# trzy/FasterRCNN

Hardware: AMD Instinct MI355X
Metric: images/sec (600x1000) Faster-RCNN VGG-16 inference (higher is better)
Workload: dtype f32 (float32 tensors and accumulation; 15 GEMM layers in the f32x3 split-operand emulation = two fp16 terms per block-scaled operand, three fp16 MFMAs per product; 0 in f32x6 = three bf16 terms, six bf16 MFMAs; the other 2 on exact-f32 MFMA; strict exact-f32 everywhere: config.strict_f32_images_per_

## Files before the change

### fasterrcnn_amd/_native.py

```python
import ctypes as C
import os

_HERE = os.path.dirname(os.path.abspath(__file__))
LIB_PATH = os.environ.get("FRCNN_LIB_PATH") or os.path.join(_HERE, "csrc", "libfrcnn_hip.so")

OK = 0
ABI_VERSION = 21
ERRORS = {0: "FRCNN_OK", -1: "FRCNN_EINVAL", -2: "FRCNN_EHIP", -3: "FRCNN_ENOMEM",
          -4: "FRCNN_EUNSUPPORTED", -5: "FRCNN_ENODEVICE"}
RELU = 1
POOL2 = 2
NUM_KCLASS = 11
KCLASS_NAMES = ("conv3x3_mfma", "conv3x3_c3", "linear_mfma", "proposals", "roi_pool", "other", "winograd_transforms",
                "winograd_gemm", "winograd_x6_transforms", "winograd_x6_gemm", "winograd_x3f")

SYMBOLS = (
    "frcnn_abi_version", "frcnn_error_string", "frcnn_last_hip_error", "frcnn_device_count",
    "frcnn_anchors", "frcnn_pack_conv3x3", "frcnn_pack_conv3x3_c3", "frcnn_pack_fc_chw_to_hwc",
    "frcnn_pack_stack_rows", "frcnn_conv3x3_c3", "frcnn_conv3x3_c3_cmax", "frcnn_conv3x3_workspace_bytes", "frcnn_conv3x3_nhwc",
    "frcnn_maxpool2x2_nhwc",
    "frcnn_linear_workspace_bytes", "frcnn_linear", "frcnn_softmax_rows", "frcnn_rpn_proposals",
    "frcnn_nms", "frcnn_roi_pool", "frcnn_roi_pool_x3t", "frcnn_detections", "frcnn_ctx_create", "frcnn_ctx_create_proposals", "frcnn_ctx_destroy",
    "frcnn_ctx_bytes", "frcnn_vgg16_forward", "frcnn_ctx_tensor", "frcnn_ctx_timing_enable",
    "frcnn_ctx_timing_read",
    "frcnn_output_block_layout", "frcnn_stream_depend", "frcnn_ctx_submit_stats", "frcnn_predict_submit", "frcnn_streams_share_queue",
    "frcnn_fold_bn_pack", "frcnn_conv_workspace_bytes", "frcnn_conv_nhwc", "frcnn_conv_nhwc_math", "frcnn_conv_nhwc_x3g", "frcnn_conv_nhwc_x3g_tickets", "frcnn_pack_conv_x3g_weights", "frcnn_x3_saturation_events", "frcnn_tensor_absmax", "frcnn_conv7x7_s2_c3",
    "frcnn_maxpool3x3_s2_nhwc", "frcnn_spatial_mean_nhwc", "frcnn_resnet_forward", "frcnn_rpn_targets",
    "frcnn_preprocess_workspace_bytes", "frcnn_preprocess",
    "frcnn_conv3x3_uses_winograd", "frcnn_resnet_block_uses_winograd", "frcnn_pack_conv3x3_winograd",
    "frcnn_pack_conv3x3_winograd_taps", "frcnn_conv3x3_winograd_workspace_bytes",
    "frcnn_conv3x3_nhwc_winograd",
    "frcnn_conv3x3_uses_winograd_fused", "frcnn_resnet_block_uses_winograd_fused", "frcnn_pack_conv3x3_winograd_fused", "frcnn_pack_conv3x3_winograd_fused_taps",
    "frcnn_conv3x3_nhwc_winograd_fused",
    "frcnn_roi_align", "frcnn_roi_align_backward",
    "frcnn_x6t_record_bytes", "frcnn_split_rows_x6t", "frcnn_gemm_x6t_workspace_bytes", "frcnn_gemm_x6t", "frcnn_split_pixels_x6t", "frcnn_split_patches3x3_x6t",
    "frcnn_conv3x3_uses_winograd_x6", "frcnn_conv3x3_winograd_x6_pack_bytes", "frcnn_pack_conv3x3_winograd_x6",
    "frcnn_conv3x3_winograd_x6_workspace_bytes", "frcnn_conv3x3_nhwc_winograd_x6",
    "frcnn_pixel_absmax", "frcnn_split_pixels_x3t", "frcnn_split_patches3x3_x3t",
    "frcnn_x3t_blob_bytes", "frcnn_pack_rows_x3t", "frcnn_conv3x3_winograd_x3_pack_bytes", "frcnn_pack_conv3x3_winograd_x3",
    "frcnn_conv3x3_winograd_x3_workspace_bytes", "frcnn_conv3x3_nhwc_winograd_x3",
    "frcnn_conv3x3_winograd_x3_fused_workspace_bytes", "frcnn_conv3x3_nhwc_winograd_x3_fused", "frcnn_conv3x3_nhwc_winograd_x3_chain",
    "frcnn_x3t_record_bytes", "frcnn_rows_scale_x3t", "frcnn_split_rows_x3t", "frcnn_gemm_x3t_workspace_bytes", "frcnn_gemm_x3t",
    "frcnn_conv3x3_nhwc_winograd_fused_maps", "frcnn_ctx_create_backbone", "frcnn_resnet_backbone", "frcnn_resnet_forward_features", "frcnn_resnet_rpn_roipool", "frcnn_ctx_create_head", "frcnn_resnet_head",
    "frcnn_label_proposals", "frcnn_gather_rows", "frcnn_rpn_loss", "frcnn_detector_loss",
    "frcnn_gemm_tn_math", "frcnn_conv3x3_wgrad_math", "frcnn_conv_wgrad_math", "frcnn_bottleneck_backward_workspace_bytes", "frcnn_bottleneck_backward",
    "frcnn_gemm_tn_workspace_bytes", "frcnn_gemm_tn", "frcnn_conv3x3_wgrad_workspace_bytes", "frcnn_conv3x3_wgrad",
    "frcnn_pack_conv3x3_dgrad", "frcnn_relu_backward", "frcnn_dropout", "frcnn_dropout_relu_backward", "frcnn_add_inplace", "frcnn_maxpool2x2_backward",
    "frcnn_roi_pool_backward_workspace_bytes", "frcnn_roi_pool_backward", "frcnn_transpose", "frcnn_sgd_step", "frcnn_sgd_step_fold",
    "frcnn_conv_wgrad_workspace_bytes", "frcnn_conv_wgrad", "frcnn_conv_dgrad_workspace_bytes", "frcnn_conv_dgrad", "frcnn_conv_dgrad_math",
    "frcnn_pack_conv_dgrad", "frcnn_scale_rows", "frcnn_bn_scale_shift", "frcnn_spatial_mean_backward",
    "frcnn_ops_roi_align", "frcnn_ops_roi_align_backward", "frcnn_ops_roi_pool", "frcnn_ops_roi_pool_backward",
    "frcnn_ops_nms_workspace_bytes", "frcnn_ops_nms",
    "frcnn_ops_ms_roi_align", "frcnn_ops_ms_roi_align_workspace_bytes", "frcnn_ops_ms_roi_align_backward",
    "frcnn_ops_half_run", "frcnn_ops_roi_align_16", "frcnn_ops_roi_align_backward_16", "frcnn_ops_roi_pool_16",
    "frcnn_ops_roi_pool_backward_16", "frcnn_ops_ms_roi_align_16", "frcnn_ops_ms_roi_align_backward_16",
    "frcnn_ops_ps_roi_pool", "frcnn_ops_ps_roi_pool_backward", "frcnn_ops_ps_roi_align", "frcnn_ops_ps_roi_align_backward",
    "frcnn_ops_ps_roi_pool_16", "frcnn_ops_ps_roi_pool_backward_16", "frcnn_ops_ps_roi_align_16", "frcnn_ops_ps_roi_align_backward_16",
    "frcnn_ops_deform_workspace_bytes", "frcnn_ops_deform_forward", "frcnn_ops_deform_backward_columns", "frcnn_ops_deform_backward_offset",
    "frcnn_ops_deform_input_plan", "frcnn_ops_deform_backward_input", "frcnn_ops_deform_backward_weight",
    "frcnn_ops_deform_roi_pool_cull_list", "frcnn_ops_deform_roi_pool_workspace_bytes", "frcnn_ops_deform_roi_pool",
    "frcnn_ops_deform_roi_pool_backward", "frcnn_ops_deform_roi_pool_16", "frcnn_ops_deform_roi_pool_backward_16",
    "frcnn_ops_box_iou_rotated", "frcnn_ops_nms_rotated", "frcnn_ops_roi_align_rotated_cull_list", "frcnn_ops_roi_align_rotated",
    "frcnn_ops_roi_align_rotated_backward", "frcnn_ops_roi_align_rotated_16", "frcnn_ops_roi_align_rotated_backward_16",
    "frcnn_ops_carafe_max_kernel", "frcnn_ops_carafe_channel_chunk", "frcnn_ops_carafe_tile_width", "frcnn_ops_carafe_tile_height",
    "frcnn_ops_carafe", "frcnn_ops_carafe_backward", "frcnn_ops_carafe_16", "frcnn_ops_carafe_backward_16",
# ... 282 lines not shown
    "frcnn_spatial_mean_nhwc": (C.c_int, [_vp, _vp, _i, _i, _i, _i, _vp]),
    "frcnn_resnet_forward": (C.c_int, [_vp, C.POINTER(ResNetWeights), C.POINTER(ForwardParams), _vp, _i, _i,
                                       _vp, _vp, _vp, _vp, _vp, _vp, _vp]),
    "frcnn_resnet_forward_features": (C.c_int, [_vp, C.POINTER(ResNetWeights), C.POINTER(ForwardParams), _vp, _i, _i,
                                                _vp, _vp, _vp, _vp, _vp, _vp, _vp]),
    "frcnn_resnet_backbone": (C.c_int, [_vp, C.POINTER(ResNetWeights), C.POINTER(ForwardParams), _vp, _i, _i, _i, _vp, _vp]),
    "frcnn_pixel_absmax": (C.c_int, [_vp, _vp, C.c_longlong, _i, _vp]),
    "frcnn_split_pixels_x3t": (C.c_int, [_vp, _vp, _vp, _vp, _i, _i, _i, _i, _i, _i, _vp]),
    "frcnn_split_patches3x3_x3t": (C.c_int, [_vp, _vp, _vp, _vp, _i, _i, _i, _i, _i, _i, _vp]),
    "frcnn_x3t_blob_bytes": (C.c_size_t, [_i, _i, _i]),
    "frcnn_pack_rows_x3t": (C.c_int, [_vp, _i, _sz, _vp, _i, _i, _i, _i, _vp]),
    "frcnn_conv3x3_winograd_x3_pack_bytes": (C.c_size_t, [_i, _i]),
    "frcnn_pack_conv3x3_winograd_x3": (C.c_int, [_vp, _vp, _i, _i, _vp]),
    "frcnn_conv3x3_winograd_x3_workspace_bytes": (C.c_size_t, [_i, _i, _i, _i, _i]),
    "frcnn_conv3x3_nhwc_winograd_x3": (C.c_int, [_vp, _vp, _vp, _vp, _i, _i, _i, _i, _i, _u, _vp, _sz, _vp]),
    "frcnn_conv3x3_winograd_x3_fused_workspace_bytes": (C.c_size_t, [_i, _i, _i]),
    "frcnn_conv3x3_nhwc_winograd_x3_fused": (C.c_int, [_vp, _vp, _vp, _vp, _i, _i, _i, _i, _i, _u, _vp, _sz, _vp]),
    "frcnn_conv3x3_nhwc_winograd_x3_chain": (C.c_int, [_vp, _vp, _vp, _vp, _i, _i, _i, _i, _i, _u, _i, _vp, _sz, _vp, _vp, _vp]),
    "frcnn_x3t_record_bytes": (C.c_size_t, [_i, _i]),
    "frcnn_rows_scale_x3t": (C.c_int, [_vp, _i, _sz, _vp, _i, _i, _i, _i, _vp]),
    "frcnn_split_rows_x3t": (C.c_int, [_vp, _i, _sz, _vp, _vp, _i, _i, _i, _i, _vp]),
    "frcnn_gemm_x3t_workspace_bytes": (C.c_size_t, [_i, _i, _i, _i]),
    "frcnn_gemm_x3t": (C.c_int, [_vp, _vp, _i, _sz, _sz, _vp, _vp, _i, _sz, _sz, _vp, _vp, _vp, _i, _sz, _i, _i, _i, _i, _u, _vp, _sz, _vp]),
    "frcnn_ctx_create_backbone": (C.c_int, [C.POINTER(C.c_void_p), _i, _i, _i]),
    "frcnn_ctx_create_head": (C.c_int, [C.POINTER(C.c_void_p), _i]),
    "frcnn_resnet_rpn_roipool": (C.c_int, [_vp, C.POINTER(ResNetWeights), C.POINTER(ForwardParams), _vp, _i, _i, _vp, _vp, _vp, _vp, _vp, _vp]),
    "frcnn_resnet_head": (C.c_int, [_vp, C.POINTER(ResNetWeights), C.POINTER(ForwardParams), _vp, _i, _vp, _vp, _vp]),
    "frcnn_conv3x3_nhwc_winograd_fused_maps": (C.c_int, [_vp, _vp, _vp, _vp, _i, _i, _i, _i, _i, _u, _vp]),
    "frcnn_label_proposals": (C.c_int, [_vp, _vp, _i, _vp, _vp, _i, _i, _f, _f, C.POINTER(C.c_float), C.POINTER(C.c_float),
                                        _vp, _vp, _vp, _vp, _vp, _vp]),
    "frcnn_gather_rows": (C.c_int, [_vp, _vp, _i, _i, _vp, _vp]),
    "frcnn_rpn_loss": (C.c_int, [_vp, _i, _i, _vp, _i, _vp, _vp, _vp, _vp]),
    "frcnn_detector_loss": (C.c_int, [_vp, _vp, _vp, _vp, _i, _i, _vp, _vp, _i, _vp]),
    "frcnn_gemm_tn_workspace_bytes": (C.c_size_t, [_i, _i, _i]),
    "frcnn_gemm_tn": (C.c_int, [_vp, _i, _vp, _i, _vp, _i, _i, _i, _i, _vp, _sz, _vp]),
    "frcnn_gemm_tn_math": (C.c_int, [_vp, _i, _vp, _i, _vp, _i, _i, _i, _i, _i, _vp, _sz, _vp]),
    "frcnn_conv3x3_wgrad_math": (C.c_int, [_vp, _vp, _vp, _i, _i, _i, _i, _i, _vp, _sz, _vp]),
    "frcnn_conv_wgrad_math": (C.c_int, [_vp, _vp, _vp, _i, _i, _i, _i, _i, _i, _i, _i, _i, _vp, _sz, _vp]),
    "frcnn_bottleneck_backward_workspace_bytes": (C.c_int, [_vp, _vp, _vp, _vp, _i, _i, _i, _i, _i, C.POINTER(C.c_size_t), C.POINTER(C.c_size_t)]),
    "frcnn_bottleneck_backward": (C.c_int, [_vp, _vp, _vp, _vp, _vp, _vp, _vp, _vp, _vp, _vp, _vp, _vp, _vp, _i, _i, _i, _i, _i, _i, _vp, _sz, _vp, _sz,
                                            _vp, _vp]),
    "frcnn_conv3x3_wgrad_workspace_bytes": (C.c_size_t, [_i, _i, _i, _i]),
    "frcnn_conv3x3_wgrad": (C.c_int, [_vp, _vp, _vp, _i, _i, _i, _i, _vp, _sz, _vp]),
    "frcnn_pack_conv3x3_dgrad": (C.c_int, [_vp, _vp, _i, _i, _vp]),
    "frcnn_conv_wgrad_workspace_bytes": (C.c_size_t, [_i] * 8),
    "frcnn_conv_wgrad": (C.c_int, [_vp, _vp, _vp, _i, _i, _i, _i, _i, _i, _i, _i, _vp, _sz, _vp]),
# ... 95 lines not shown
```

### fasterrcnn_amd/csrc/api.hip

```cpp
#include "common.h"
#include <algorithm>
#include <cmath>
#include <cstring>
#include <string>
#include <vector>
#include <new>

namespace frcnn {

static thread_local std::string g_hip_error;
void set_hip_error(hipError_t e) { g_hip_error = hipGetErrorString(e); }

static size_t align_up(size_t v, size_t a) { return (v + a - 1) / a * a; }

struct EventRec { int cls; hipEvent_t start, stop; };

}

using namespace frcnn;

struct frcnn_ctx {
    int max_h = 0, max_w = 0, max_rois = 0, max_images = 0;
    int max_fh = 0, max_fw = 0, a_cap = 0, pre_cap = 0;
    void* slab = nullptr;
// ... 267 lines not shown
    if (!d_a || !d_inv_scale) return FRCNN_EINVAL;
    return launch_rows_scale_x3t(d_a, lda, a_batch_floats, d_inv_scale, rows, rows_padded, K, batches, as_stream(stream));
}

int frcnn_split_rows_x3t(const float* d_a, int lda, size_t a_batch_floats, const float* d_inv_scale, void* d_rec, int rows, int rows_padded,
                         int K, int batches, void* stream)
{
    if (!d_a || !d_rec || !d_inv_scale) return FRCNN_EINVAL;
    return launch_split_rows_x3t(d_a, lda, a_batch_floats, d_inv_scale, d_rec, rows, rows_padded, K, batches, as_stream(stream));
}

size_t frcnn_gemm_x3t_workspace_bytes(int M, int N, int K, int batches) { return gemm_x3t_workspace_bytes(M, N, K, batches); }

int frcnn_gemm_x3t(const void* d_a_rec, const float* d_a_inv, int a_rows, size_t a_batch_bytes, size_t a_inv_batch_floats,
                   const void* d_b_rec, const float* d_b_inv, int b_rows, size_t b_batch_bytes, size_t b_inv_batch_floats,
                   const float* d_bias, const float* d_residual, float* d_c, int ldc, size_t c_batch_floats, int M, int N, int K,
                   int batches, unsigned flags, void* d_ws, size_t ws_bytes, void* stream)
{
    return launch_gemm_x3t(d_a_rec, d_a_inv, a_rows, a_batch_bytes, a_inv_batch_floats, d_b_rec, d_b_inv, b_rows, b_batch_bytes,
                           b_inv_batch_floats, d_bias, d_residual, d_c, ldc, c_batch_floats, M, N, K, batches, flags, d_ws, ws_bytes,
                           as_stream(stream));
}

size_t frcnn_conv3x3_winograd_x3_fused_workspace_bytes(int n_maps, int H, int W)
{
    return n_maps > 0 && H > 0 && W > 0 ? conv3x3_winograd_x3_fused_workspace_bytes(n_maps, H, W) : 0;
}

int frcnn_conv3x3_nhwc_winograd_x3_fused(const float* d_x, const void* d_blob, const float* d_bias, float* d_y, int n_maps, int H, int W,
                                         int cin, int cout, unsigned flags, void* d_ws, size_t ws_bytes, void* stream)
{
    if (!d_x || !d_blob || !d_bias || !d_y) return FRCNN_EINVAL;
    return launch_conv3x3_winograd_x3_fused(d_x, d_blob, d_bias, d_y, n_maps, H, W, cin, cout, flags, d_ws, ws_bytes, as_stream(stream));
}

int frcnn_pixel_absmax(const float* d_x, float* d_cmax, long long pixels, int c, void* stream)
{
    if (!d_x || !d_cmax) return FRCNN_EINVAL;
    return launch_pixel_absmax(d_x, d_cmax, pixels, c, as_stream(stream));
}

int frcnn_split_pixels_x3t(const float* d_x, const float* d_cmax, void* d_rec, float* d_inv_scale, int n_maps, int H, int W, int c, int stride,
                           int rows_padded, void* stream)
{
    if (!d_x || !d_rec) return FRCNN_EINVAL;
    return launch_split_pixels_x3t(d_x, d_cmax, d_rec, d_inv_scale, n_maps, H, W, c, stride, rows_padded, as_stream(stream));
// ... 1024 lines not shown

    const int R_ = p->post_nms;
    const bool fc_x6t = p->fc_math_mode == FRCNN_FC_F32X6T;
    const bool fc_x3t = p->fc_math_mode == FRCNN_FC_F32X3T;
    if (fc_x6t || fc_x3t) { rc = ensure_fc_records(c, s); if (rc) return rc; }
    if (fc_x3t) {
        const int rr = c->rec_rows;
        const size_t w1rec = x3t_record_bytes(4096, 49 * 512), w2rec = x3t_record_bytes(4096, 4096);
        const float* w1inv = reinterpret_cast<const float*>(reinterpret_cast<const unsigned char*>(w->fc1_w) + w1rec);
        const float* w2inv = reinterpret_cast<const float*>(reinterpret_cast<const unsigned char*>(w->fc2_w) + w2rec);
        if (p->roi_op == FRCNN_ROI_ALIGN) {
            STEP(4, launch_roi_align(c->fm, fh, fw, 512, d_props, d_counts + 2, R_, 7, 1.0f / 16.0f, p->roi_sampling_ratio, 0, c->roi_out, s));
            STEP(2, launch_rows_scale_x3t(c->roi_out, 49 * 512, 0, c->roi_inv, R_, rr, 49 * 512, 1, s));
            STEP(2, launch_split_rows_x3t(c->roi_out, 49 * 512, 0, c->roi_inv, c->roi_rec, R_, rr, 49 * 512, 1, s));
        } else {
            STEP(4, launch_roi_pool_x3t(c->fm, fh, fw, 512, d_props, d_counts + 2, R_, 7, 1.0f / 16.0f,
                                        fm_cmax_ready ? const_cast<float*>(fm_cmax_ready) : c->fm_cmax, c->roi_inv, c->roi_rec, rr, s, fm_cmax_ready != nullptr));
        }
        STEP(2, launch_gemm_x3t(c->roi_rec, c->roi_inv, rr, 0, 0, w->fc1_w, w1inv, 4096, 0, 0, w->fc1_b, nullptr, c->fc1_out, 4096, 0, R_, 4096,
                                49 * 512, 1, R, c->lin_ws, c->lin_ws_bytes, s, 0));
        STEP(2, launch_rows_scale_x3t(c->fc1_out, 4096, 0, c->fc1_inv, R_, rr, 4096, 1, s));
        STEP(2, launch_split_rows_x3t(c->fc1_out, 4096, 0, c->fc1_inv, c->fc1_rec, R_, rr, 4096, 1, s));
        STEP(2, launch_gemm_x3t(c->fc1_rec, c->fc1_inv, rr, 0, 0, w->fc2_w, w2inv, 4096, 0, 0, w->fc2_b, nullptr, c->fc2_out, 4096, 0, R_, 4096,
                                4096, 1, R, c->lin_ws, c->lin_ws_bytes, s, 2));
    } else
    if (fc_x6t) {
        const int rr = c->rec_rows;
        if (p->roi_op == FRCNN_ROI_ALIGN) {
            STEP(4, launch_roi_align(c->fm, fh, fw, 512, d_props, d_counts + 2, R_, 7, 1.0f / 16.0f, p->roi_sampling_ratio, 0, c->roi_out, s));
            STEP(2, launch_split_rows_x6t(c->roi_out, 49 * 512, 0, c->roi_rec, R_, rr, 49 * 512, 1, s));
        } else {
            STEP(4, launch_roi_pool_x6t(c->fm, fh, fw, 512, d_props, d_counts + 2, R_, 7, 1.0f / 16.0f, c->roi_rec, rr, s));
        }
        static const int fc_tiles = []() { const char* e = frcnn_knob("FRCNN_FC_TILES"); return e ? atoi(e) : 0; }();
        STEP(2, launch_gemm_x6t(c->roi_rec, rr, 0, w->fc1_w, 4096, 0, w->fc1_b, nullptr, c->fc1_out, 4096, 0, R_, 4096, 49 * 512, 1, R,
                                c->lin_ws, c->lin_ws_bytes, s, fc_tiles));
        STEP(2, launch_split_rows_x6t(c->fc1_out, 4096, 0, c->fc1_rec, R_, rr, 4096, 1, s));
        STEP(2, launch_gemm_x6t(c->fc1_rec, rr, 0, w->fc2_w, 4096, 0, w->fc2_b, nullptr, c->fc2_out, 4096, 0, R_, 4096, 4096, 1, R,
                                c->lin_ws, c->lin_ws_bytes, s, fc_tiles));
    } else
    {
        if (p->roi_op == FRCNN_ROI_ALIGN) {
            STEP(4, launch_roi_align(c->fm, fh, fw, 512, d_props, d_counts + 2, R_, 7, 1.0f / 16.0f, p->roi_sampling_ratio, 0, c->roi_out, s));
        } else {
            STEP(4, launch_roi_pool(c->fm, fh, fw, 512, d_props, d_counts + 2, R_, 7, 1.0f / 16.0f, c->roi_out, s));
        }
        STEP(2, launch_linear(c->roi_out, 49 * 512, w->fc1_w, w->fc1_b, c->fc1_out, 4096, R_, 4096, 49 * 512, R,
// ... 641 lines not shown
```

### fasterrcnn_amd/csrc/gemm_x3t.hip

```cpp
#include "x3t.h"

namespace frcnn {

typedef _Float16 hx_f16x8 __attribute__((ext_vector_type(8)));

#ifndef HX_ABLATE
#define HX_ABLATE 0
#endif
__global__ __launch_bounds__(256)
void rows_scale_x3t_kernel(const float* __restrict__ a, int lda, size_t a_batch, float* __restrict__ inv_scale, int R, int rows_padded,
                           int K, int batches)
{
    const int lane = threadIdx.x & 63;
    const long long wave = (long long)blockIdx.x * 4 + (threadIdx.x >> 6);
    if (wave >= (long long)batches * rows_padded) return;
    const int row = (int)(wave % rows_padded), batch = (int)(wave / rows_padded);
    float mx = 0.f;
    if (row < R) {
        const float* src = a + (size_t)batch * a_batch + (size_t)row * lda;
        for (int k = 4 * lane; k < K; k += 256) {
            const f32x4 v = *reinterpret_cast<const f32x4*>(src + k);
            mx = fmaxf(fmaxf(mx, fmaxf(fabsf(v[0]), fabsf(v[1]))), fmaxf(fabsf(v[2]), fabsf(v[3])));
        }
    }
// ... 179 lines not shown
    int nchunks, chunks_per_split, splits, batches;
    int mtiles, ntiles;
    int relu;
    int total;
};

template <int WTM, int WTN, int WVM, int WVN, int NSUB>
struct HxCfg {
    static constexpr int NW = WVM * WVN, THREADS = 64 * NW;
    static constexpr int ARB = WVM * WTM, BRB = WVN * WTN;
    static constexpr int BM = 32 * ARB, BN = 32 * BRB;
    static constexpr int A_BYTES = ARB * HX_RB, B_BYTES = BRB * HX_RB;
    static constexpr int STAGE1 = A_BYTES + B_BYTES;
    static constexpr int STAGE = NSUB * STAGE1;
    static constexpr int NBUF = NSUB == 1 ? 3 : 2;
    static constexpr int DIST = NBUF - 1;
    static constexpr size_t LDS_BYTES = NBUF * (size_t)STAGE;
    static constexpr int NPA = ARB * 2, NPB = BRB * 2, NP = NPA + NPB;
    static constexpr int PPW = (NSUB * NP + NW - 1) / NW;
};

typedef __attribute__((address_space(3))) void* hx_lds_ptr;

template <int WTM, int WTN, int WVM, int WVN, int NSUB>
__global__ __launch_bounds__(64 * WVM * WVN, 2)
void gemm_x3t_kernel(const HxParams p)
{
    using C = HxCfg<WTM, WTN, WVM, WVN, NSUB>;
    extern __shared__ __attribute__((aligned(16))) unsigned char smem_hx[];
    const int tid = threadIdx.x, lane = tid & 63;
    const int wave = __builtin_amdgcn_readfirstlane(tid >> 6);
    const int wm = wave / WVN, wn = wave % WVN;

    int bid = blockIdx.x;
    {
        const int q = p.total >> 3, r = p.total & 7, xcd = bid & 7, idx = bid >> 3;
        bid = (xcd < r ? xcd * (q + 1) : r * (q + 1) + (xcd - r) * q) + idx;
    }
    const int nt = bid % p.ntiles;
    int t = bid / p.ntiles;
    const int mt = t % p.mtiles;
    t /= p.mtiles;
    const int split = t % p.splits;
    const int batch = t / p.splits;

    const int c_begin = split * p.chunks_per_split;
    int c_end = c_begin + p.chunks_per_split;
    if (c_end > p.nchunks) c_end = p.nchunks;
    const int nst = (c_end - c_begin) / NSUB;

    const size_t a_chunk = (size_t)p.a_rbt * HX_RB, b_chunk = (size_t)p.b_rbt * HX_RB;
    const unsigned char* ag = p.a + (size_t)batch * p.a_batch + (size_t)mt * C::A_BYTES + (size_t)c_begin * a_chunk + lane * 16;
    const unsigned char* bg = p.b + (size_t)batch * p.b_batch + (size_t)nt * C::B_BYTES + (size_t)c_begin * b_chunk + lane * 16;

    auto issue_stage = [&](int s, int buf) {
        const unsigned char* as = ag + (size_t)s * NSUB * a_chunk;
        const unsigned char* bs = bg + (size_t)s * NSUB * b_chunk;
        unsigned char* ldsb = smem_hx + buf * C::STAGE;
#pragma unroll
        for (int i = 0; i < C::PPW; ++i) {
            int q = wave + C::NW * i;
            q = q < NSUB * C::NP ? q : NSUB * C::NP - 1;
            const int sub = q / C::NP, r = q - sub * C::NP;
            const unsigned char* src = r < C::NPA ? as + sub * a_chunk + r * HX_PIECE : bs + sub * b_chunk + (r - C::NPA) * HX_PIECE;
            __builtin_amdgcn_global_load_lds(src, (hx_lds_ptr)(ldsb + sub * C::STAGE1 + r * HX_PIECE), 16, 0, 0);
        }
    };
    f32x16 acc[WTM][WTN];
#pragma unroll
    for (int i = 0; i < WTM; ++i)
#pragma unroll
        for (int j = 0; j < WTN; ++j)
#pragma unroll
            for (int r = 0; r < 16; ++r) acc[i][j][r] = 0.f;

    hx_f16x8 ah[WTM], al[WTM], bh[WTN], bl[WTN];
#pragma unroll
    for (int i = 0; i < WTM; ++i)
#pragma unroll
        for (int e = 0; e < 8; ++e) al[i][e] = (_Float16)0.f;
#pragma unroll
    for (int j = 0; j < WTN; ++j)
#pragma unroll
        for (int e = 0; e < 8; ++e) bh[j][e] = (_Float16)0.f;

#ifndef HX_NO_SCHED
#define HX_NO_SCHED 0
#endif
#define HX_SGB(mask, n) __builtin_amdgcn_sched_group_barrier(mask, n, 0)
#define HX_TERM(A, B)                                                                                  \
    _Pragma("unroll") for (int i = 0; i < WTM; ++i)                                                     \
        _Pragma("unroll") for (int j = 0; j < WTN; ++j)                                                 \
            if (!(HX_ABLATE & 2)) acc[i][j] = __builtin_amdgcn_mfma_f32_32x32x16_f16(B[j], A[i], acc[i][j], 0, 0, 0);

#ifdef HX_CLOCKS
    unsigned long long clk0 = 0, real0 = 0, clk1 = 0, real1 = 0;
    const unsigned long long real_entry = __builtin_amdgcn_s_memrealtime();
#endif
    if (nst > 0) {
        issue_stage(0, 0);
        if (C::DIST == 2) issue_stage(nst > 1 ? 1 : 0, 1);
        asm volatile("s_waitcnt vmcnt(%0)" ::"n"((C::DIST - 1) * C::PPW) : "memory");
        __builtin_amdgcn_s_barrier();
        int cur = 0;
        const int a_off = wm * WTM * HX_RB + lane * 16;
        const int b_off = C::A_BYTES + wn * WTN * HX_RB + lane * 16;
#ifdef HX_CLOCKS
        clk0 = __builtin_readcyclecounter(); real0 = __builtin_amdgcn_s_memrealtime();
#endif
        for (int s = 0; s < nst; ++s) {
            const int nxt = C::NBUF == 3 ? (cur == 0 ? 2 : cur - 1) : (cur ^ 1);
#pragma unroll
            for (int sub = 0; sub < NSUB; ++sub) {
                const unsigned char* at = smem_hx + cur * C::STAGE + sub * C::STAGE1 + a_off;
                const unsigned char* bt = smem_hx + cur * C::STAGE + sub * C::STAGE1 + b_off;
                if (!(HX_ABLATE & 16) || s == 0) {
#pragma unroll
                for (int i = 0; i < WTM; ++i) ah[i] = *reinterpret_cast<const hx_f16x8*>(at + i * HX_RB);
#pragma unroll
                for (int j = 0; j < WTN; ++j) bl[j] = *reinterpret_cast<const hx_f16x8*>(bt + j * HX_RB + HX_PIECE);
                }
                if (sub == 0 && !(HX_ABLATE & 1)) issue_stage(s + C::DIST < nst ? s + C::DIST : nst - 1, nxt);
                HX_TERM(al, bh)
                HX_TERM(ah, bl)
                if (!(HX_ABLATE & 16) || s == 0) {
#pragma unroll
                for (int j = 0; j < WTN; ++j) bh[j] = *reinterpret_cast<const hx_f16x8*>(bt + j * HX_RB);
#pragma unroll
                for (int i = 0; i < WTM; ++i) al[i] = *reinterpret_cast<const hx_f16x8*>(at + i * HX_RB + HX_PIECE);
                }
                HX_TERM(ah, bh)
#if !HX_NO_SCHED && !HX_ABLATE
// ... 2 lines not shown
                if (sub == 0) {
                    _Pragma("unroll") for (int q = 0; q < (PW < NT ? PW : NT); ++q) { HX_SGB(0x008, 1); HX_SGB(0x010, 1); }
                    if (PW > NT) HX_SGB(0x010, PW - NT);
                    if (NT > PW) HX_SGB(0x008, NT - PW);
                } else {
                    HX_SGB(0x008, NT);
                }
                _Pragma("unroll") for (int q = 0; q < (NF < NT ? NF : NT); ++q) { HX_SGB(0x008, 1); HX_SGB(0x100, 1); }
                if (NF > NT) HX_SGB(0x100, NF - NT);
                if (NT > NF) HX_SGB(0x008, NT - NF);
                HX_SGB(0x008, NT);
#endif
            }
            __builtin_amdgcn_sched_barrier(0);
            asm volatile("s_waitcnt vmcnt(%0) lgkmcnt(0)" ::"n"((C::DIST - 1) * C::PPW) : "memory");
            __builtin_amdgcn_s_barrier();
            cur = cur == C::NBUF - 1 ? 0 : cur + 1;
            __builtin_amdgcn_sched_barrier(0);
        }
#ifdef HX_CLOCKS
        clk1 = __builtin_readcyclecounter(); real1 = __builtin_amdgcn_s_memrealtime();
#endif
        HX_TERM(al, bh)
        asm volatile("s_waitcnt vmcnt(0)" ::: "memory");
    }
#undef HX_TERM
#undef HX_SGB

    const bool direct = p.splits == 1;
    float* dst;
    int ldd;
    if (direct) { dst = p.c + (size_t)batch * p.c_batch; ldd = p.ldc; }
    else        { dst = p.ws + ((size_t)split * p.batches + batch) * (size_t)p.M * p.N; ldd = p.N; }
    const int m_base = mt * C::BM + 32 * WTM * wm + (lane & 31);
    const int n_base = nt * C::BN + 32 * WTN * wn + 4 * (lane >> 5);
    const float* ainv = p.a_inv + (size_t)batch * p.a_inv_batch;
    const float* binv = p.b_inv + (size_t)batch * p.b_inv_batch;
#pragma unroll
    for (int i = 0; i < WTM; ++i) {
        const int m = m_base + 32 * i;
        if (m >= p.M) continue;
        const float sa = ainv[m];
        float* row = dst + (size_t)m * ldd;
#pragma unroll
        for (int j = 0; j < WTN; ++j) {
#pragma unroll
            for (int g = 0; g < 4; ++g) {
                const int n = n_base + 32 * j + 8 * g;
                if (n >= p.N) continue;
                const f32x4 sb = *reinterpret_cast<const f32x4*>(binv + n);
                f32x4 v;
#pragma unroll
                for (int e = 0; e < 4; ++e) v[e] = (acc[i][j][4 * g + e] * sa) * sb[e];
                if (direct && p.bias != nullptr) v = v + *reinterpret_cast<const f32x4*>(p.bias + n);
                if (direct && p.residual != nullptr)
                    v = v + *reinterpret_cast<const f32x4*>(p.residual + (size_t)batch * p.c_batch + (size_t)m * ldd + n);
                if (direct && p.relu) {
#pragma unroll
                    for (int e = 0; e < 4; ++e) v[e] = fmaxf(v[e], 0.f);
                }
                if (HX_ABLATE & 4) asm volatile("" ::"v"(v));
                else *reinterpret_cast<f32x4*>(row + n) = v;
            }
        }
    }
#ifdef HX_CLOCKS
    if (lane == 0 && p.ws != nullptr) {
        const unsigned long long real_exit = __builtin_amdgcn_s_memrealtime();
        float* o = p.ws + ((size_t)blockIdx.x * C::NW + wave) * 8;
        o[0] = (float)(clk1 - clk0); o[1] = (float)(real1 - real0); o[2] = (float)(real0 - real_entry); o[3] = (float)(real_exit - real1);
        o[4] = (float)nst; o[5] = (float)(real_entry & 0xFFFFFF); o[6] = (float)(real_exit & 0xFFFFFF); o[7] = 1.0f;
    }
#endif
}

size_t x3t_record_bytes(int rows_padded, int K) { return (size_t)(K / 16) * (rows_padded / 32) * HX_RB; }

int launch_rows_scale_x3t(const float* a, int lda, size_t a_batch_floats, float* inv_scale, int R, int rows_padded, int K, int batches,
                          hipStream_t s)
{
    if (R < 1 || rows_padded < R || rows_padded % 32 != 0 || K < 16 || K % 16 != 0 || lda < K || lda % 4 != 0 || batches < 1)
        return FRCNN_EINVAL;
    const long long waves = (long long)batches * rows_padded;
    const long long blocks = (waves + 3) / 4;
    if (blocks > 0x7fffffffLL) return FRCNN_EINVAL;
    hipLaunchKernelGGL(rows_scale_x3t_kernel, dim3((unsigned)blocks), dim3(256), 0, s, a, lda, a_batch_floats, inv_scale, R, rows_padded, K,
                       batches);
// ... 31 lines not shown
    return check_launch();
}

int launch_split_patches3x3_x3t(const float* x, const float* cmax, void* rec, float* inv, int N, int H, int W, int C, int stride,
                                int rows_padded, hipStream_t s)
{
    if (N < 1 || H < 1 || W < 1 || C < 16 || C % 16 != 0 || stride < 1 || stride > 2 || rows_padded % 32 != 0 || !cmax || !inv) return FRCNN_EINVAL;
    const int Ho = (H - 1) / stride + 1, Wo = (W - 1) / stride + 1;
    const long long R = (long long)N * Ho * Wo;
    if (R > rows_padded || R > 0x7fffffffLL) return FRCNN_EINVAL;
    const long long waves = (long long)(9 * C / 16) * (rows_padded / 32);
    hipLaunchKernelGGL(split_patches3x3_x3t_kernel, dim3((unsigned)((waves + 3) / 4)), dim3(256), 0, s, x, cmax,
                       static_cast<unsigned char*>(rec), inv, H, W, Ho, Wo, C, stride, (int)R, rows_padded / 32, 9 * C / 16);
    return check_launch();
}

struct HxPlan { int cfg, mtiles, ntiles, splits, chunks_per_split; };

static HxPlan plan_gemm_x3t(int M, int N, int K, int batches, int tiles_mode = -1)
{
    HxPlan pl;
    const int chunks = K / 16;
    static const int env_force = []() { const char* e = frcnn_knob("FRCNN_HX_CFG"); return e ? atoi(e) : -1; }();
    const int mode = tiles_mode >= 0 ? tiles_mode : gemm_x6t_get_tiles();
    const int force = (env_force >= 0 && tiles_mode < 0) ? env_force : (mode == 1 ? 0 : mode == 2 ? 1 : -1);
    const long long u0 = (long long)cdiv(M, 320) * cdiv(N, 256) * batches;
    const long long u1 = (long long)cdiv(M, 160) * cdiv(N, 128) * batches;
    int splits0 = 1;
    while (u0 * splits0 * 2 <= 256 && chunks / (splits0 * 2) >= 8) splits0 *= 2;
    const double c0 = (double)((u0 * splits0 + 255) / 256) * 1920.0 / splits0 + (splits0 > 1 ? 600.0 : 0.0);
    int splits1 = 1;
    while (u1 * splits1 * 2 <= 256 && chunks / (splits1 * 2) >= 8) splits1 *= 2;
    const double c1 = (double)((u1 * splits1 + 255) / 256) * 480.0 / 0.85 / splits1 + (splits1 > 1 ? 600.0 : 0.0);
    pl.cfg = (force == 0 || force == 1) ? force : (c1 < c0 ? 1 : 0);
    static const bool big_unsplit = frcnn_knob("FRCNN_HX_BIG_UNSPLIT") != nullptr;
    if (big_unsplit && force < 0 && pl.cfg == 1 && splits1 == 1) { pl.cfg = 0; splits0 = 1; }
    int splits = pl.cfg == 1 ? splits1 : splits0;
    if (splits > chunks) splits = chunks;
    pl.mtiles = pl.cfg == 1 ? cdiv(M, 160) : cdiv(M, 320);
    pl.ntiles = pl.cfg == 1 ? cdiv(N, 128) : cdiv(N, 256);
    pl.chunks_per_split = cdiv(chunks, splits);
    pl.splits = cdiv(chunks, pl.chunks_per_split);
    return pl;
}

size_t gemm_x3t_workspace_bytes(int M, int N, int K, int batches)
// ... 20 lines not shown
    const HxPlan pl = plan_gemm_x3t(M, N, K, batches, tiles_mode);
    if (pl.splits > 1 && (ws == nullptr || ws_bytes < (size_t)pl.splits * batches * M * N * sizeof(float))) return FRCNN_EINVAL;
    HxParams p;
    p.a = static_cast<const unsigned char*>(a_rec);
    p.b = static_cast<const unsigned char*>(b_rec);
    p.a_inv = a_inv; p.b_inv = b_inv;
    p.c = c;
    p.ws = static_cast<float*>(ws);
    p.bias = bias;
    p.residual = residual;
    p.a_batch = a_batch_bytes; p.b_batch = b_batch_bytes; p.c_batch = c_batch_floats;
    p.a_inv_batch = a_inv_batch; p.b_inv_batch = b_inv_batch;
    p.a_rbt = a_rows / 32; p.b_rbt = b_rows / 32;
    p.M = M; p.N = N; p.ldc = ldc;
    p.nchunks = K / 16; p.chunks_per_split = pl.chunks_per_split; p.splits = pl.splits; p.batches = batches;
    p.mtiles = pl.mtiles; p.ntiles = pl.ntiles;
    p.relu = (flags & FRCNN_RELU) ? 1 : 0;
    const long long total = (long long)pl.mtiles * pl.ntiles * batches * pl.splits;
    if (total > 0x7fffffffLL) return FRCNN_EINVAL;
    p.total = (int)total;
    static const int env_nsub = []() { const char* e = frcnn_knob("FRCNN_HX_NSUB"); return e ? atoi(e) : 0; }();
    const int last = p.nchunks - (pl.splits - 1) * pl.chunks_per_split;
    const bool even = pl.chunks_per_split % 2 == 0 && last % 2 == 0;
    const int nsub = !even ? 1 : (env_nsub == 1 || env_nsub == 2) ? env_nsub : (pl.chunks_per_split >= 64 ? 2 : 1);
#define HX_LAUNCH(TM, TN, VM, VN, NS)                                                                          \
    do {                                                                                                      \
        using C = HxCfg<TM, TN, VM, VN, NS>;                                                                    \
        auto kern = gemm_x3t_kernel<TM, TN, VM, VN, NS>;                                                        \
        FRCNN_MAX_LDS_ONCE(kern, C::LDS_BYTES);                                                                 \
        hipLaunchKernelGGL(kern, dim3((unsigned)total), dim3(C::THREADS), C::LDS_BYTES, s, p);                  \
    } while (0)
    if (pl.cfg == 1) { if (nsub == 2) HX_LAUNCH(5, 1, 1, 4, 2); else HX_LAUNCH(5, 1, 1, 4, 1); }
    else             { if (nsub == 2) HX_LAUNCH(5, 2, 2, 4, 2); else HX_LAUNCH(5, 2, 2, 4, 1); }
#undef HX_LAUNCH
    int rc = check_launch();
    if (rc || pl.splits == 1) return rc;
    return launch_gemm_x6t_reduce(static_cast<const float*>(ws), bias, residual, c, ldc, c_batch_floats, M, N, batches, pl.splits, p.relu, s);
}

}
```

### fasterrcnn_amd/csrc/x3t.h

```cpp
#pragma once
#include "common.h"

namespace frcnn {

static constexpr int HX_PIECE = 1024;
static constexpr int HX_RB = 2 * HX_PIECE;

__device__ __forceinline__ unsigned hx_pack2(_Float16 a, _Float16 b)
{
    return (unsigned)__builtin_bit_cast(unsigned short, a) | ((unsigned)__builtin_bit_cast(unsigned short, b) << 16);
}

__device__ __forceinline__ void hx_split8(const float (&v)[8], uint4& ph, uint4& pl)
{
    _Float16 hi[8], lo[8];
#pragma unroll
    for (int j = 0; j < 8; ++j) {
        const float vj = v[j] > 65504.f ? 65504.f : (v[j] < -65504.f ? -65504.f : v[j]);
        hi[j] = (_Float16)vj;
        lo[j] = (_Float16)(vj - (float)hi[j]);
    }
    ph = make_uint4(hx_pack2(hi[0], hi[1]), hx_pack2(hi[2], hi[3]), hx_pack2(hi[4], hi[5]), hx_pack2(hi[6], hi[7]));
    pl = make_uint4(hx_pack2(lo[0], lo[1]), hx_pack2(lo[2], lo[3]), hx_pack2(lo[4], lo[5]), hx_pack2(lo[6], lo[7]));
}

__device__ __forceinline__ void hx_row_scale(float mx, float& mult, float& inv)
{
    int e = 0;
    if (mx > 0.f) {
// ... 12 lines not shown
```

### include/frcnn_hip.h

```cpp
#ifndef FRCNN_HIP_H
#define FRCNN_HIP_H

#include <stddef.h>
#include <stdint.h>

#ifdef __cplusplus
extern "C" {
#endif

#define FRCNN_OK            0
#define FRCNN_EINVAL       -1
#define FRCNN_EHIP         -2
#define FRCNN_ENOMEM       -3
#define FRCNN_EUNSUPPORTED -4
#define FRCNN_ENODEVICE    -5

#define FRCNN_ABI_VERSION 21

#define FRCNN_RELU   1u
#define FRCNN_POOL2  2u
#define FRCNN_X3G_WSPLIT 0x800u

int         frcnn_abi_version(void);
const char* frcnn_error_string(int code);
// ... 64 lines not shown
int frcnn_pack_rows_x3t(const float* d_a, int lda, size_t a_batch_floats, void* d_blob, int rows, int rows_padded, int K, int batches,
                        void* stream);
size_t frcnn_conv3x3_winograd_x3_pack_bytes(int cout, int cin);
int frcnn_pack_conv3x3_winograd_x3(const float* d_u_f32, void* d_blob, int cout, int cin, void* stream);
size_t frcnn_conv3x3_winograd_x3_workspace_bytes(int n_maps, int H, int W, int cin, int cout);
int frcnn_conv3x3_nhwc_winograd_x3(const float* d_x, const void* d_blob, const float* d_bias, float* d_y, int n_maps, int H, int W, int cin,
                                   int cout, unsigned flags, void* d_ws, size_t ws_bytes, void* stream);
size_t frcnn_conv3x3_winograd_x3_fused_workspace_bytes(int n_maps, int H, int W);
int frcnn_conv3x3_nhwc_winograd_x3_fused(const float* d_x, const void* d_blob, const float* d_bias, float* d_y, int n_maps, int H, int W,
                                         int cin, int cout, unsigned flags, void* d_ws, size_t ws_bytes, void* stream);
int frcnn_conv3x3_nhwc_winograd_x3_chain(const float* d_x, const void* d_blob, const float* d_bias, float* d_y, int n_maps, int H, int W, int cin,
                                         int cout, unsigned flags, int one_launch, void* d_ws, size_t ws_bytes, const float* d_cmax_in,
                                         float* d_cmax_out, void* stream);
size_t frcnn_x3t_record_bytes(int rows_padded, int K);
int frcnn_rows_scale_x3t(const float* d_a, int lda, size_t a_batch_floats, float* d_inv_scale, int rows, int rows_padded, int K, int batches,
                         void* stream);
int frcnn_split_rows_x3t(const float* d_a, int lda, size_t a_batch_floats, const float* d_inv_scale, void* d_rec, int rows, int rows_padded,
                         int K, int batches, void* stream);
size_t frcnn_gemm_x3t_workspace_bytes(int M, int N, int K, int batches);
int frcnn_gemm_x3t(const void* d_a_rec, const float* d_a_inv, int a_rows, size_t a_batch_bytes, size_t a_inv_batch_floats,
                   const void* d_b_rec, const float* d_b_inv, int b_rows, size_t b_batch_bytes, size_t b_inv_batch_floats,
                   const float* d_bias, const float* d_residual, float* d_c, int ldc, size_t c_batch_floats, int M, int N, int K,
                   int batches, unsigned flags, void* d_ws, size_t ws_bytes, void* stream);

int frcnn_split_pixels_x6t(const float* d_x, void* d_rec, int N, int H, int W, int C, int stride, int rows_padded, void* stream);
int frcnn_conv3x3_uses_winograd_x6(int cin, int cout);
size_t frcnn_conv3x3_winograd_x6_pack_bytes(int cout, int cin);
int frcnn_pack_conv3x3_winograd_x6(const float* d_w_oihw, const float* d_row_scale, void* d_u_rec, int cout, int cin, void* stream);
size_t frcnn_conv3x3_winograd_x6_workspace_bytes(int n_maps, int H, int W, int cin, int cout);
int frcnn_conv3x3_nhwc_winograd_x6(const float* d_x, const void* d_u_rec, const float* d_bias, float* d_y, int n_maps, int H, int W, int cin,
                                   int cout, unsigned flags, void* d_ws, size_t ws_bytes, void* stream);
int frcnn_split_patches3x3_x6t(const float* d_x, void* d_rec, int N, int H, int W, int C, int stride, int rows_padded, void* stream);
int frcnn_maxpool2x2_nhwc(const float* d_x, float* d_y, int H, int W, int c, void* stream);

int frcnn_fold_bn_pack(const float* d_w_oihw, const float* d_gamma, const float* d_beta,
                       const float* d_mean, const float* d_var, float eps, int cout, int cin, int ksize,
                       float* d_w_packed, float* d_b_packed, void* stream);
size_t frcnn_conv_workspace_bytes(int N, int H, int W, int cin, int cout, int ksize, int stride, int pad);
int frcnn_conv_nhwc(const float* d_x, const float* d_w_packed, const float* d_bias, const float* d_residual,
                    float* d_y, int N, int H, int W, int cin, int cout, int ksize, int stride, int pad,
                    unsigned flags, void* d_ws, size_t ws_bytes, void* stream);
int frcnn_conv7x7_s2_c3(const float* d_x_chw, const float* d_w_packed, const float* d_bias, float* d_y,
                        int H, int W, int cout, unsigned flags, void* stream);
int frcnn_maxpool3x3_s2_nhwc(const float* d_x, float* d_y, int H, int W, int c, void* stream);
int frcnn_spatial_mean_nhwc(const float* d_x, float* d_y, int N, int H, int W, int c, void* stream);

// ... 459 lines not shown
```

Before: 980.3.

## Add 16x16x32 f16 MFMA path for x3t GEMM and use it for fc2

Adds a K32 variant of the x3t split-fp16 GEMM kernel that issues 16x16x32 f16 MFMAs over both 16-k chunks of a stage, using 4-wide accumulators and a new fragment-offset layout. It software-pipelines the global-to-LDS loads between MFMA groups. The fc2 layer call switches to tiles mode 4 to select this path, and a new API entry point exposes the tile mode. This gives higher MFMA throughput per instruction and better overlap, at the cost of more accumulator registers and a new epilogue mapping.

```diff
diff --git a/fasterrcnn_amd/_native.py b/fasterrcnn_amd/_native.py
--- a/fasterrcnn_amd/_native.py
+++ b/fasterrcnn_amd/_native.py
@@ -41,6 +41,7 @@
     "frcnn_conv3x3_winograd_x3_workspace_bytes", "frcnn_conv3x3_nhwc_winograd_x3",
     "frcnn_conv3x3_winograd_x3_fused_workspace_bytes", "frcnn_conv3x3_nhwc_winograd_x3_fused", "frcnn_conv3x3_nhwc_winograd_x3_chain",
     "frcnn_x3t_record_bytes", "frcnn_rows_scale_x3t", "frcnn_split_rows_x3t", "frcnn_gemm_x3t_workspace_bytes", "frcnn_gemm_x3t",
+    "frcnn_gemm_x3t_tiles", "frcnn_x3t_frag16_offset",
     "frcnn_conv3x3_nhwc_winograd_fused_maps", "frcnn_ctx_create_backbone", "frcnn_resnet_backbone", "frcnn_resnet_forward_features", "frcnn_resnet_rpn_roipool", "frcnn_ctx_create_head", "frcnn_resnet_head",
     "frcnn_label_proposals", "frcnn_gather_rows", "frcnn_rpn_loss", "frcnn_detector_loss",
     "frcnn_gemm_tn_math", "frcnn_conv3x3_wgrad_math", "frcnn_conv_wgrad_math", "frcnn_bottleneck_backward_workspace_bytes", "frcnn_bottleneck_backward",
@@ -369,6 +370,8 @@
     "frcnn_split_rows_x3t": (C.c_int, [_vp, _i, _sz, _vp, _vp, _i, _i, _i, _i, _vp]),
     "frcnn_gemm_x3t_workspace_bytes": (C.c_size_t, [_i, _i, _i, _i]),
     "frcnn_gemm_x3t": (C.c_int, [_vp, _vp, _i, _sz, _sz, _vp, _vp, _i, _sz, _sz, _vp, _vp, _vp, _i, _sz, _i, _i, _i, _i, _u, _vp, _sz, _vp]),
+    "frcnn_gemm_x3t_tiles": (C.c_int, [_vp, _vp, _i, _sz, _sz, _vp, _vp, _i, _sz, _sz, _vp, _vp, _vp, _i, _sz, _i, _i, _i, _i, _u, _vp, _sz, _vp, _i]),
+    "frcnn_x3t_frag16_offset": (C.c_int, [_i, _i, _i]),
     "frcnn_ctx_create_backbone": (C.c_int, [C.POINTER(C.c_void_p), _i, _i, _i]),
     "frcnn_ctx_create_head": (C.c_int, [C.POINTER(C.c_void_p), _i]),
     "frcnn_resnet_rpn_roipool": (C.c_int, [_vp, C.POINTER(ResNetWeights), C.POINTER(ForwardParams), _vp, _i, _i, _vp, _vp, _vp, _vp, _vp, _vp]),
diff --git a/fasterrcnn_amd/csrc/api.hip b/fasterrcnn_amd/csrc/api.hip
--- a/fasterrcnn_amd/csrc/api.hip
+++ b/fasterrcnn_amd/csrc/api.hip
@@ -1,4 +1,5 @@
 #include "common.h"
+#include "x3t.h"
 #include <algorithm>
 #include <cmath>
 #include <cstring>
@@ -313,6 +314,23 @@
                            as_stream(stream));
 }
 
+int frcnn_gemm_x3t_tiles(const void* d_a_rec, const float* d_a_inv, int a_rows, size_t a_batch_bytes, size_t a_inv_batch_floats,
+                         const void* d_b_rec, const float* d_b_inv, int b_rows, size_t b_batch_bytes, size_t b_inv_batch_floats,
+                         const float* d_bias, const float* d_residual, float* d_c, int ldc, size_t c_batch_floats, int M, int N, int K,
+                         int batches, unsigned flags, void* d_ws, size_t ws_bytes, void* stream, int tiles_mode)
+{
+    if (tiles_mode < -1 || tiles_mode > 4) return FRCNN_EINVAL;
+    return launch_gemm_x3t(d_a_rec, d_a_inv, a_rows, a_batch_bytes, a_inv_batch_floats, d_b_rec, d_b_inv, b_rows, b_batch_bytes,
+                           b_inv_batch_floats, d_bias, d_residual, d_c, ldc, c_batch_floats, M, N, K, batches, flags, d_ws, ws_bytes,
+                           as_stream(stream), tiles_mode);
+}
+
+int frcnn_x3t_frag16_offset(int lane, int half, int stage1_bytes)
+{
+    if (lane < 0 || lane > 63 || half < 0 || half > 1 || stage1_bytes < HX_RB || stage1_bytes % HX_RB != 0) return -1;
+    return hx_frag16_offset(lane, stage1_bytes) + 256 * half;
+}
+
 size_t frcnn_conv3x3_winograd_x3_fused_workspace_bytes(int n_maps, int H, int W)
 {
     return n_maps > 0 && H > 0 && W > 0 ? conv3x3_winograd_x3_fused_workspace_bytes(n_maps, H, W) : 0;
@@ -1383,7 +1401,7 @@
         STEP(2, launch_rows_scale_x3t(c->fc1_out, 4096, 0, c->fc1_inv, R_, rr, 4096, 1, s));
         STEP(2, launch_split_rows_x3t(c->fc1_out, 4096, 0, c->fc1_inv, c->fc1_rec, R_, rr, 4096, 1, s));
         STEP(2, launch_gemm_x3t(c->fc1_rec, c->fc1_inv, rr, 0, 0, w->fc2_w, w2inv, 4096, 0, 0, w->fc2_b, nullptr, c->fc2_out, 4096, 0, R_, 4096,
-                                4096, 1, R, c->lin_ws, c->lin_ws_bytes, s, 2));
+                                4096, 1, R, c->lin_ws, c->lin_ws_bytes, s, 4));
     } else
     if (fc_x6t) {
         const int rr = c->rec_rows;
diff --git a/fasterrcnn_amd/csrc/gemm_x3t.hip b/fasterrcnn_amd/csrc/gemm_x3t.hip
--- a/fasterrcnn_amd/csrc/gemm_x3t.hip
+++ b/fasterrcnn_amd/csrc/gemm_x3t.hip
@@ -225,10 +225,11 @@
 
 typedef __attribute__((address_space(3))) void* hx_lds_ptr;
 
-template <int WTM, int WTN, int WVM, int WVN, int NSUB>
+template <int WTM, int WTN, int WVM, int WVN, int NSUB, bool K32 = false>
 __global__ __launch_bounds__(64 * WVM * WVN, 2)
 void gemm_x3t_kernel(const HxParams p)
 {
+    static_assert(!K32 || NSUB == 2, "the 16x16x32 body reads both chunks of a 32-k stage");
     using C = HxCfg<WTM, WTN, WVM, WVN, NSUB>;
     extern __shared__ __attribute__((aligned(16))) unsigned char smem_hx[];
     const int tid = threadIdx.x, lane = tid & 63;
@@ -269,21 +270,31 @@
             __builtin_amdgcn_global_load_lds(src, (hx_lds_ptr)(ldsb + sub * C::STAGE1 + r * HX_PIECE), 16, 0, 0);
         }
     };
-    f32x16 acc[WTM][WTN];
+    constexpr int MT = 2 * WTM, NT = 2 * WTN;
+    f32x16 acc[K32 ? 1 : WTM][K32 ? 1 : WTN];
+    f32x4 acc4[K32 ? MT : 1][K32 ? NT : 1];
+    if constexpr (K32) {
+#pragma unroll
+        for (int i = 0; i < MT; ++i)
+#pragma unroll
+            for (int j = 0; j < NT; ++j) acc4[i][j] = f32x4{0.f, 0.f, 0.f, 0.f};
+    } else {
 #pragma unroll
     for (int i = 0; i < WTM; ++i)
 #pragma unroll
         for (int j = 0; j < WTN; ++j)
 #pragma unroll
             for (int r = 0; r < 16; ++r) acc[i][j][r] = 0.f;
-
-    hx_f16x8 ah[WTM], al[WTM], bh[WTN], bl[WTN];
-#pragma unroll
-    for (int i = 0; i < WTM; ++i)
+    }
+
+    constexpr int FM = K32 ? MT : WTM, FN = K32 ? NT : WTN;
+    hx_f16x8 ah[FM], al[FM], bh[FN], bl[FN];
+#pragma unroll
+    for (int i = 0; i < FM; ++i)
 #pragma unroll
         for (int e = 0; e < 8; ++e) al[i][e] = (_Float16)0.f;
 #pragma unroll
-    for (int j = 0; j < WTN; ++j)
+    for (int j = 0; j < FN; ++j)
 #pragma unroll
         for (int e = 0; e < 8; ++e) bh[j][e] = (_Float16)0.f;
 
@@ -311,6 +322,85 @@
 #ifdef HX_CLOCKS
         clk0 = __builtin_readcyclecounter(); real0 = __builtin_amdgcn_s_memrealtime();
 #endif
+        if constexpr (K32) {
+        constexpr int DF = NT >= 4 ? 3 : 5, TG = NT >= 4 ? 1 : 2;
+        static_assert(DF < MT && MT % TG == 0, "tiles");
+        hx_f16x8 bn[NT];
+        constexpr int PWA = NSUB * C::NPA / C::NW, PWB = NSUB * C::NPB / C::NW, PW = PWA + PWB, PWD = (PW + DF - 1) / DF;
+        static_assert(NSUB * C::NPA % C::NW == 0 && NSUB * C::NPB % C::NW == 0 && PW == C::PPW, "pieces per wave");
+        const int frag = hx_frag16_offset(lane, C::STAGE1);
+        const int a_off16 = wm * WTM * HX_RB + frag;
+        const int b_off16 = C::A_BYTES + wn * WTN * HX_RB + frag;
+#define HX_FENCE __builtin_amdgcn_sched_barrier(0)
+#define HX_FRAG16(base, t, term) *reinterpret_cast<const hx_f16x8*>((base) + ((t) >> 1) * HX_RB + ((t) & 1) * 256 + (term) * HX_PIECE)
+#define HX_ROW16(A, B, i)                                                                                       \
+    _Pragma("unroll") for (int j = 0; j < NT; ++j)                                                               \
+        if (!(HX_ABLATE & 2)) acc4[i][j] = __builtin_amdgcn_mfma_f32_16x16x32_f16(B[j], A[i], acc4[i][j], 0, 0, 0);
+        for (int s = 0; s < nst; ++s) {
+            const int nxt = cur ^ 1;
+            const int sn = s + 1 < nst ? s + 1 : nst - 1;
+            const unsigned char* at = smem_hx + cur * C::STAGE + a_off16;
+            const unsigned char* bt = smem_hx + cur * C::STAGE + b_off16;
+            const unsigned char* as = ag + (size_t)sn * NSUB * a_chunk;
+            const unsigned char* bs = bg + (size_t)sn * NSUB * b_chunk;
+            unsigned char* ldsb = smem_hx + nxt * C::STAGE;
+#pragma unroll
+            for (int i = 0; i < TG; ++i) ah[i] = HX_FRAG16(at, i, 0);
+#pragma unroll
+            for (int j = 0; j < NT; ++j) bl[j] = HX_FRAG16(bt, j, 1);
+#pragma unroll
+            for (int j = 0; j < NT; ++j) bn[j] = HX_FRAG16(bt, j, 0);
+#pragma unroll
+            for (int i = 0; i < TG; ++i) al[i] = HX_FRAG16(at, i, 1);
+            HX_FENCE;
+#pragma unroll
+            for (int d = 0; d < DF; ++d) {
+#pragma unroll
+                for (int i = 0; i < PW; ++i) {
+                    if (i / PWD == d && !(HX_ABLATE & 1)) {
+                        const bool is_a = i < PWA;
+                        const int q = wave + C::NW * (is_a ? i : i - PWA);
+                        const int sub = q / (is_a ? C::NPA : C::NPB), r = q - sub * (is_a ? C::NPA : C::NPB);
+                        const unsigned char* src = is_a ? as + sub * a_chunk + r * HX_PIECE : bs + sub * b_chunk + r * HX_PIECE;
+                        __builtin_amdgcn_global_load_lds(src, (hx_lds_ptr)(ldsb + sub * C::STAGE1 + (is_a ? 0 : C::A_BYTES) + r * HX_PIECE), 16, 0, 0);
+                    }
+                }
+                HX_ROW16(al, bh, MT - DF + d)
+                HX_FENCE;
+            }
+#pragma unroll
+            for (int j = 0; j < NT; ++j) bh[j] = bn[j];
+#pragma unroll
+            for (int g = 0; g < MT; g += TG) {
+                if (!(HX_ABLATE & 2)) acc4[g][0] = __builtin_amdgcn_mfma_f32_16x16x32_f16(bl[0], ah[g], acc4[g][0], 0, 0, 0);
+                HX_FENCE;
+#pragma unroll
+                for (int i = g + TG; i < g + 2 * TG && i < MT; ++i) { ah[i] = HX_FRAG16(at, i, 0); al[i] = HX_FRAG16(at, i, 1); }
+                HX_FENCE;
+#pragma unroll
+                for (int i = g; i < g + TG; ++i) {
+#pragma unroll
+                    for (int j = i == g ? 1 : 0; j < NT; ++j)
+                        if (!(HX_ABLATE & 2)) acc4[i][j] = __builtin_amdgcn_mfma_f32_16x16x32_f16(bl[j], ah[i], acc4[i][j], 0, 0, 0);
+                    HX_ROW16(ah, bh, i)
+                    if (i < MT - DF) HX_ROW16(al, bh, i)
+                }
+                HX_FENCE;
+            }
+            asm volatile("s_waitcnt vmcnt(0) lgkmcnt(0)" ::: "memory");
+            __builtin_amdgcn_s_barrier();
+            cur ^= 1;
+            HX_FENCE;
+        }
+#ifdef HX_CLOCKS
+        clk1 = __builtin_readcyclecounter(); real1 = __builtin_amdgcn_s_memrealtime();
+#endif
+#pragma unroll
+        for (int d = 0; d < DF; ++d) HX_ROW16(al, bh, MT - DF + d)
+#undef HX_ROW16
+#undef HX_FRAG16
+#undef HX_FENCE
+        } else {
         for (int s = 0; s < nst; ++s) {
             const int nxt = C::NBUF == 3 ? (cur == 0 ? 2 : cur - 1) : (cur ^ 1);
 #pragma unroll
@@ -359,6 +449,7 @@
         clk1 = __builtin_readcyclecounter(); real1 = __builtin_amdgcn_s_memrealtime();
 #endif
         HX_TERM(al, bh)
+        }
         asm volatile("s_waitcnt vmcnt(0)" ::: "memory");
     }
 #undef HX_TERM
@@ -373,6 +464,35 @@
     const int n_base = nt * C::BN + 32 * WTN * wn + 4 * (lane >> 5);
     const float* ainv = p.a_inv + (size_t)batch * p.a_inv_batch;
     const float* binv = p.b_inv + (size_t)batch * p.b_inv_batch;
+    if constexpr (K32) {
+        const int m16 = mt * C::BM + 32 * WTM * wm + (lane & 15);
+        const int n16 = nt * C::BN + 32 * WTN * wn + 4 * (lane >> 4);
+#pragma unroll
+        for (int i = 0; i < MT; ++i) {
+            const int m = m16 + 16 * i;
+            if (m >= p.M) continue;
+            const float sa = ainv[m];
+            float* row = dst + (size_t)m * ldd;
+#pragma unroll
+            for (int j = 0; j < NT; ++j) {
+                const int n = n16 + 16 * j;
+                if (n >= p.N) continue;
+                const f32x4 sb = *reinterpret_cast<const f32x4*>(binv + n);
+                f32x4 v;
+#pragma unroll
+                for (int e = 0; e < 4; ++e) v[e] = (acc4[i][j][e] * sa) * sb[e];
+                if (direct && p.bias != nullptr) v = v + *reinterpret_cast<const f32x4*>(p.bias + n);
+                if (direct && p.residual != nullptr)
+                    v = v + *reinterpret_cast<const f32x4*>(p.residual + (size_t)batch * p.c_batch + (size_t)m * ldd + n);
+                if (direct && p.relu) {
+#pragma unroll
+                    for (int e = 0; e < 4; ++e) v[e] = fmaxf(v[e], 0.f);
+                }
+                if (HX_ABLATE & 4) asm volatile("" ::"v"(v));
+                else *reinterpret_cast<f32x4*>(row + n) = v;
+            }
+        }
+    } else {
 #pragma unroll
     for (int i = 0; i < WTM; ++i) {
         const int m = m_base + 32 * i;
@@ -400,6 +520,7 @@
                 else *reinterpret_cast<f32x4*>(row + n) = v;
             }
         }
+    }
     }
 #ifdef HX_CLOCKS
     if (lane == 0 && p.ws != nullptr) {
@@ -477,6 +598,7 @@
     HxPlan pl;
     const int chunks = K / 16;
     static const int env_force = []() { const char* e = frcnn_knob("FRCNN_HX_CFG"); return e ? atoi(e) : -1; }();
+    if (tiles_mode == 3 || tiles_mode == 4) tiles_mode -= 2;
     const int mode = tiles_mode >= 0 ? tiles_mode : gemm_x6t_get_tiles();
     const int force = (env_force >= 0 && tiles_mode < 0) ? env_force : (mode == 1 ? 0 : mode == 2 ? 1 : -1);
     const long long u0 = (long long)cdiv(M, 320) * cdiv(N, 256) * batches;
@@ -543,16 +665,17 @@
     static const int env_nsub = []() { const char* e = frcnn_knob("FRCNN_HX_NSUB"); return e ? atoi(e) : 0; }();
     const int last = p.nchunks - (pl.splits - 1) * pl.chunks_per_split;
     const bool even = pl.chunks_per_split % 2 == 0 && last % 2 == 0;
-    const int nsub = !even ? 1 : (env_nsub == 1 || env_nsub == 2) ? env_nsub : (pl.chunks_per_split >= 64 ? 2 : 1);
-#define HX_LAUNCH(TM, TN, VM, VN, NS)                                                                          \
+    const bool k32 = (tiles_mode == 3 || tiles_mode == 4) && even;
+    const int nsub = !even ? 1 : k32 ? 2 : (env_nsub == 1 || env_nsub == 2) ? env_nsub : (pl.chunks_per_split >= 64 ? 2 : 1);
+#define HX_LAUNCH(TM, TN, VM, VN, NS, ...)                                                                     \
     do {                                                                                                      \
         using C = HxCfg<TM, TN, VM, VN, NS>;                                                                    \
-        auto kern = gemm_x3t_kernel<TM, TN, VM, VN, NS>;                                                        \
+        auto kern = gemm_x3t_kernel<TM, TN, VM, VN, NS, ##__VA_ARGS__>;                                         \
         FRCNN_MAX_LDS_ONCE(kern, C::LDS_BYTES);                                                                 \
         hipLaunchKernelGGL(kern, dim3((unsigned)total), dim3(C::THREADS), C::LDS_BYTES, s, p);                  \
     } while (0)
-    if (pl.cfg == 1) { if (nsub == 2) HX_LAUNCH(5, 1, 1, 4, 2); else HX_LAUNCH(5, 1, 1, 4, 1); }
-    else             { if (nsub == 2) HX_LAUNCH(5, 2, 2, 4, 2); else HX_LAUNCH(5, 2, 2, 4, 1); }
+    if (pl.cfg == 1) { if (k32) HX_LAUNCH(5, 1, 1, 4, 2, true); else if (nsub == 2) HX_LAUNCH(5, 1, 1, 4, 2); else HX_LAUNCH(5, 1, 1, 4, 1); }
+    else             { if (k32) HX_LAUNCH(5, 2, 2, 4, 2, true); else if (nsub == 2) HX_LAUNCH(5, 2, 2, 4, 2); else HX_LAUNCH(5, 2, 2, 4, 1); }
 #undef HX_LAUNCH
     int rc = check_launch();
     if (rc || pl.splits == 1) return rc;
diff --git a/fasterrcnn_amd/csrc/x3t.h b/fasterrcnn_amd/csrc/x3t.h
--- a/fasterrcnn_amd/csrc/x3t.h
+++ b/fasterrcnn_amd/csrc/x3t.h
@@ -5,6 +5,11 @@
 
 static constexpr int HX_PIECE = 1024;
 static constexpr int HX_RB = 2 * HX_PIECE;
+
+__host__ __device__ constexpr int hx_frag16_offset(int lane, int stage1)
+{
+    return (lane >> 5) * stage1 + (((lane >> 4) & 1) * 32 + (lane & 15)) * 16;
+}
 
 __device__ __forceinline__ unsigned hx_pack2(_Float16 a, _Float16 b)
 {
diff --git a/include/frcnn_hip.h b/include/frcnn_hip.h
--- a/include/frcnn_hip.h
+++ b/include/frcnn_hip.h
@@ -110,6 +110,11 @@
                    const void* d_b_rec, const float* d_b_inv, int b_rows, size_t b_batch_bytes, size_t b_inv_batch_floats,
                    const float* d_bias, const float* d_residual, float* d_c, int ldc, size_t c_batch_floats, int M, int N, int K,
                    int batches, unsigned flags, void* d_ws, size_t ws_bytes, void* stream);
+int frcnn_gemm_x3t_tiles(const void* d_a_rec, const float* d_a_inv, int a_rows, size_t a_batch_bytes, size_t a_inv_batch_floats,
+                         const void* d_b_rec, const float* d_b_inv, int b_rows, size_t b_batch_bytes, size_t b_inv_batch_floats,
+                         const float* d_bias, const float* d_residual, float* d_c, int ldc, size_t c_batch_floats, int M, int N, int K,
+                         int batches, unsigned flags, void* d_ws, size_t ws_bytes, void* stream, int tiles_mode);
+int frcnn_x3t_frag16_offset(int lane, int half, int stage1_bytes);
 
 int frcnn_split_pixels_x6t(const float* d_x, void* d_rec, int N, int H, int W, int C, int stride, int rows_padded, void* stream);
 int frcnn_conv3x3_uses_winograd_x6(int cin, int cout);
```

Result: no change. 983.7 (median of 4 runs) (+0.3%).
